# wustl-cig/FLAIR

Measured on AMD Instinct MI355X. Metric: restored frames/sec at 256x256, 16-frame clip, 250-step DDIM, higher is better.
Workload: dtype bf16

## Files before the change

flair_amd/csrc/conv.hip:

```cpp
#include <type_traits>

#include "common.h"
#include "mfma_tile.h"

namespace {

struct ConvArgs {
    const void* x[4];
    int segC[4];
    int segLd[4];
    int nseg;
    const void* w;
    const float* bias;
    const void* res0;
    const void* res1;
    int res0Ld, res1Ld;
    void* y;
    int yLd;
    int T, H, W;
    int KT, KH, KW;
    int Cout, CinTot;
    int act;
    float outScale;
    long P;
    int nPixTiles, nCoTiles;
    int tFast;
    unsigned segBytes[4];
    unsigned wBytes;
    float* part;
    int splitK;
    const float* fbias;
    int fbiasLd;
    int stride;
    int tapShift;
    int reflect;
    float actParam;
    int actPeriod;
    int Hin, Win;
    int esz;
};

__device__ __forceinline__ int lds_off(int row, int chunk) {
    return row * 64 + ((chunk ^ ((row >> 2) & 3)) << 4);
}

__device__ __forceinline__ int staged_row(int id) {
    const int g = id >> 3;
    return (g >> 2) * 8 + (g & 3) + 4 * ((id >> 2) & 1);
}

template <typename E>
__device__ __forceinline__ void store_quad(const ConvArgs& a, long p, int co, float v0, float v1, float v2, float v3) {
    if (co >= a.Cout) return;
    float v[4] = {v0, v1, v2, v3};
    if (a.bias) {
        const float4 b = *reinterpret_cast<const float4*>(a.bias + co);
// ... 187 lines not shown
        const unsigned cofs = (unsigned)(cb * BKE) * ESZ;
#pragma unroll
        for (int i = 0; i < HI; ++i) {
            const unsigned off = hpix[i] >= 0 ? (unsigned)hpix[i] * ld + cofs + hq[i] : FLAIR_OOB;
            hr[i] = buf_load16(xr, off);
        }
        const unsigned kofs = (unsigned)((dt + pt) * 9 * a.CinTot + segOff + cb * BKE) * ESZ;
#pragma unroll
        for (int i = 0; i < WI; ++i) wr[i] = buf_load16(wrs, woff[i] == FLAIR_OOB ? FLAIR_OOB : woff[i] + kofs);
    };
    auto advance = [&]() {
        ++cb;
        if (cb * BKE >= a.segC[seg]) {
            cb = 0;
            segOff += a.segC[seg];
            if (++seg >= a.nseg) {
                seg = 0;
                segOff = 0;
                ++dt;
                while (dt <= pt && !dt_valid(dt)) ++dt;
            }
        }
    };
    auto write_lds = [&](const uint4 (&hr)[HI], const uint4 (&wr)[WI]) {
#pragma unroll
        for (int i = 0; i < HI; ++i) {
            const int id = i * NT + tid;
            const int row = staged_row(id);
            if (row < HALO_ROWS) *reinterpret_cast<uint4*>(sh + row * PITCH + (id & 3) * 16) = hr[i];
        }
#pragma unroll
        for (int i = 0; i < WI; ++i) {
            const int id = i * NT + tid;
            if (id < W_PIECES) *reinterpret_cast<uint4*>(sw + staged_row(id) * PITCH + (id & 3) * 16) = wr[i];
        }
    };
    int nValidDt = 0;
    for (int d = -pt; d <= pt; ++d) nValidDt += dt_valid(d) ? 1 : 0;
    const int nch = nValidDt * (a.CinTot / BKE);

    f32x16 acc[RPW][2];
#pragma unroll
    for (int j = 0; j < RPW; ++j)
#pragma unroll
        for (int i = 0; i < 2; ++i)
#pragma unroll
            for (int r = 0; r < 16; ++r) acc[j][i][r] = 0.f;

    auto compute = [&]() {
        const char* hb = sh + ((wave * RPW * HW_) + lr) * PITCH;
        const char* wb0 = sw + (lr * 9) * PITCH;
        const char* wb1 = sw + ((lr + 32) * 9) * PITCH;
        uint4 fa0[2][2], fa1[2][2], fb[2][RPW][2];
        auto load_tap = [&](int set, int tap9) {
// ... 221 lines not shown
    auto issue = [&]() {
        const unsigned ld = (unsigned)a.segLd[seg] * ESZ;
        const char* frame = reinterpret_cast<const char*>(a.x[seg]) + (size_t)(t + dt) * a.H * a.W * ld;
        const __amdgpu_buffer_rsrc_t xr = make_rsrc(frame, a.segBytes[seg]);
        const unsigned cofs = (unsigned)(cb * BKE) * ESZ;
#pragma unroll
        for (int i = 0; i < HI; ++i)
            hreg[i] = buf_load16(xr, hpix[i] >= 0 ? (unsigned)hpix[i] * ld + cofs + hq[i] : FLAIR_OOB);
        const unsigned kofs = (unsigned)((dt + pt) * 9 * a.CinTot + segOff + cb * BKE) * ESZ;
#pragma unroll
        for (int i = 0; i < WI; ++i) wreg[i] = buf_load16(wrs, woff[i] == FLAIR_OOB ? FLAIR_OOB : woff[i] + kofs);
        ++cb;
        if (cb * BKE >= a.segC[seg]) {
            cb = 0;
            segOff += a.segC[seg];
            if (++seg >= a.nseg) {
                seg = 0;
                segOff = 0;
                ++dt;
                while (dt <= pt && !dt_valid(dt)) ++dt;
            }
        }
    };
    auto write_lds = [&](int stage) {
        char* sh = smem + stage * STAGE_BYTES;
        char* sw = sh + HALO_BYTES;
#pragma unroll
        for (int i = 0; i < HI; ++i) {
            const int id = i * NT + tid;
            const int row = staged_row(id);
            if (row < HALO_ROWS) *reinterpret_cast<uint4*>(sh + row * PITCH + (id & 3) * 16) = hreg[i];
        }
#pragma unroll
        for (int i = 0; i < WI; ++i) {
            const int id = i * NT + tid;
            if (id < W_PIECES) *reinterpret_cast<uint4*>(sw + staged_row(id) * PITCH + (id & 3) * 16) = wreg[i];
        }
    };
    int nValidDt = 0;
    for (int d = -pt; d <= pt; ++d) nValidDt += dt_valid(d) ? 1 : 0;
    const int nch = nValidDt * (a.CinTot / BKE);

    f32x16 acc[2];
#pragma unroll
    for (int i = 0; i < 2; ++i)
#pragma unroll
        for (int r = 0; r < 16; ++r) acc[i][r] = 0.f;

    const int ck = 16 * Mma<E>::chunk(kh2, lh);
    auto compute = [&](int stage) {
        const char* sh = smem + stage * STAGE_BYTES;
        const char* hb = sh + ((rp * HW_) + lr) * PITCH + ck;
        const char* wb0 = sh + HALO_BYTES + (lr * 9) * PITCH + ck;
        uint4 fa[2][2], fb[2];
        auto load_tap = [&](int set, int tap9) {
            const int kh = tap9 / 3, kw = tap9 % 3;
// ... 134 lines not shown
    constexpr int KSTEPS = 2;
    constexpr int TH = NW * RPW, HWP = 34;
    constexpr int HALO_ROWS = (TH + 2) * HWP;
    constexpr int HALO_INSTR = (HALO_ROWS + 15) / 16;
    constexpr int W_INSTR = 64 * 9 / 16;
    constexpr int HALO_BYTES = HALO_INSTR * 1024;
    constexpr int STAGE_BYTES = HALO_BYTES + W_INSTR * 1024;
    constexpr int NSLOT = (HALO_INSTR + W_INSTR + NW - 1) / NW;
    constexpr int BIAS_OFF = NSTAGE * STAGE_BYTES + NW * 1024;
    extern __shared__ __attribute__((aligned(16))) char smem[];

    const int tid = threadIdx.x, lane = tid & 63;
    const int wave = __builtin_amdgcn_readfirstlane(tid >> 6);
    const int lr = lane & 31, lh = lane >> 5;
    const int taps = a.KT * 9, pt = a.KT / 2;
    const int chunksPerTap = a.CinTot / 32;
    const int H = a.H, W = a.W, T = a.T;

    const int xcd = blockIdx.x & 7, slot = blockIdx.x >> 3, slotsPerXcd = gridDim.x >> 3;
    const int tilesW = W / 32, tilesH = H / TH, nCoTiles = a.nCoTiles;
    auto tile_at = [&](int i, DmaTile& tl) -> bool {
        const int inXcd = slot + i * slotsPerXcd;
        const int id = xcd * tilesPerXcd + inXcd;
        if (inXcd >= tilesPerXcd || id >= nTiles) return false;
        int rest = id;
        tl.co0 = (rest % nCoTiles) * 64;
        rest /= nCoTiles;
        if (a.tFast) {
            tl.t = rest % T;
            rest /= T;
            tl.w0 = (rest % tilesW) * 32;
// ... 35 lines not shown
    const u32x4_t wdesc = make_desc(a.w, a.wBytes);
    struct Walk {
        int dt, seg, cb, segOff, j;
    };
    auto dt_at = [&](int t, int j) { return a.tFast ? (j + a.KT * T - t) % a.KT - pt : j - pt; };
    auto walk_first = [&](int t, Walk& wk) {
        wk.j = 0; wk.seg = 0; wk.cb = 0; wk.segOff = 0;
        while (wk.j < a.KT && (unsigned)(t + dt_at(t, wk.j)) >= (unsigned)T) ++wk.j;
        wk.dt = dt_at(t, wk.j);
    };
    auto walk_next = [&](int t, Walk& wk) {
        ++wk.cb;
        if (wk.cb * 32 >= a.segC[wk.seg]) {
            wk.cb = 0;
            wk.segOff += a.segC[wk.seg];
            if (++wk.seg >= a.nseg) {
                wk.seg = 0;
                wk.segOff = 0;
                ++wk.j;
                while (wk.j < a.KT && (unsigned)(t + dt_at(t, wk.j)) >= (unsigned)T) ++wk.j;
                wk.dt = dt_at(t, wk.j);
            }
        }
    };
    auto chunks_of = [&](int t) {
        int n = 0;
        for (int d = -pt; d <= pt; ++d) n += (unsigned)(t + d) < (unsigned)T ? 1 : 0;
        return n * chunksPerTap;
    };
    auto issue = [&](const DmaTile& tl, const Walk& wk, int stage) {
        const unsigned ld = (unsigned)a.segLd[wk.seg] * 2u;
// ... 338 lines not shown
    using E = bf16_t;
    constexpr int NW = 8, HWP = 34;
    constexpr int HINSTR = 22, HIMG = HINSTR * 1024, WINSTR = 36, SLOT = WINSTR * 1024;
    constexpr int HR = 3, WR = 2;
    constexpr int RING = HR * HIMG, BIAS = RING + WR * SLOT;
    constexpr int NH = (HINSTR + NW - 1) / NW, NWS = (WINSTR + NW - 1) / NW;
    extern __shared__ __attribute__((aligned(16))) char smem[];
    const int tid = threadIdx.x, lane = tid & 63;
    const int wave = __builtin_amdgcn_readfirstlane(tid >> 6);
    const int lr = lane & 31, lh = lane >> 5;
    const int lrow = lane >> 2, lchunk = lane & 3;
    const int tilesW = a.W / 32, perFrame = tilesW * (a.H / 8);
    const int bid = xcd_remap(blockIdx.x, gridDim.x);
    const int t = bid / perFrame, tile = bid - t * perFrame;
    const int h0 = (tile / tilesW) * 8, w0 = (tile % tilesW) * 32;
    const int nS = a.CinTot / 32;

    const u32x4_t wdesc = make_desc(a.w, a.wBytes);
    const u32x4_t bdesc = make_desc(a.bias, a.bias ? (unsigned)a.Cout * 4u : 0u);
    dma16(bdesc, (unsigned)(lane * 16), (unsigned)BIAS);
    unsigned hpix[NH], hpiece[NH];
#pragma unroll
    for (int i = 0; i < NH; ++i) dma_halo_coords((wave * NH + i) % HINSTR, lrow, lchunk, 10, h0, w0, a.H, a.W, hpix[i], hpiece[i]);
    unsigned wlane[NWS];
#pragma unroll
    for (int i = 0; i < NWS; ++i) {
        const int id = (wave * NWS + i) % WINSTR;
        const int row = id * 16 + lrow, tap9 = row >> 6, co = row & 63;
        wlane[i] = co < a.Cout ? (unsigned)((co * 9 + tap9) * a.CinTot) * 2u + (unsigned)((lchunk ^ ((co >> 2) & 3)) << 4) : FLAIR_OOB;
    }
    int hseg = 0, hcb = 0;
    auto issue_halo = [&](int slot) {
        const unsigned ld = (unsigned)a.segLd[hseg] * 2u;
        const u32x4_t xdesc = make_desc(reinterpret_cast<const char*>(a.x[hseg]) + (size_t)t * a.H * a.W * ld, a.segBytes[hseg]);
        const unsigned cofs = (unsigned)(hcb * 64);
#pragma unroll
        for (int i = 0; i < NH; ++i) {
            const int k = (wave * NH + i) % HINSTR;
            dma16(xdesc, hpix[i] == 0xffffffffu ? FLAIR_OOB : hpix[i] * ld + cofs + hpiece[i], (unsigned)(slot * HIMG + k * 1024));
        }
        if (++hcb * 32 >= a.segC[hseg]) {
            hcb = 0;
            ++hseg;
        }
    };
    auto issue_w = [&](int s_) {
#pragma unroll
        for (int i = 0; i < NWS; ++i) {
            const int id = (wave * NWS + i) % WINSTR;
            dma16(wdesc, wlane[i] == FLAIR_OOB ? FLAIR_OOB : wlane[i] + (unsigned)(s_ * 64), (unsigned)(RING + (s_ % WR) * SLOT + id * 1024));
        }
    };
    issue_halo(0);
    issue_w(0);
    if (nS > 1) {
        issue_halo(1);
        issue_w(1);
    }
    if (nS > 2) issue_halo(2);

    unsigned aoff[2], boff[3][2];
    dma_frag_offsets(lr, lh, wave * HWP, aoff, boff);
    f32x16 acc[2];
    auto compute = [&](int wslot, int hslot) { dma_tap_loop(smem + RING + wslot * SLOT, smem + hslot * HIMG, aoff, boff, acc, dma_no_hook{}); };

    const long prow = ((long)t * a.H + h0 + wave) * a.W + w0;
// ... 111 lines not shown
        xvalid[i] = p < a.P;
        if (!xvalid[i]) p = 0;
        int w_ = (int)(p % a.W);
        long q = p / a.W;
        xw[i] = w_;
        xh[i] = (int)(q % a.H);
        xt[i] = (int)(q / a.H);
    }
    const int taps = a.KT * a.KH * a.KW;
    const int pt = a.KT / 2, ph = a.KH / 2, pw = a.KW / 2;
    const int tFirst = (int)(p0 / ((long)a.H * a.W));
    const int tileFrames = (int)((TP + (long)a.H * a.W - 1) / ((long)a.H * a.W)) + 1;

    uint4 xreg[PD][XR], wreg[PD][WR];

    const int nkAll = taps * (a.CinTot / BKE);
    const int ks0 = (int)((long)blockIdx.y * nkAll / a.splitK);
    const int ks1 = (int)((long)(blockIdx.y + 1) * nkAll / a.splitK);
    int tap = ks0 / (a.CinTot / BKE), seg = 0, cb = ks0 % (a.CinTot / BKE), segOff = 0;
    while (cb * BKE >= a.segC[seg]) {
        cb -= a.segC[seg] / BKE;
        segOff += a.segC[seg];
        ++seg;
    }
    int dw = tap % a.KW - pw, dh = (tap / a.KW) % a.KH - ph, dt = tap / (a.KW * a.KH) - pt;

    const __amdgpu_buffer_rsrc_t wrs = make_rsrc(a.w, a.wBytes);
    constexpr unsigned ESZ = sizeof(E);
    auto issue_loads = [&](int set) {
        const int ld = a.segLd[seg];
        int fb = tFirst + dt;
        fb = fb < 0 ? 0 : (fb >= a.T ? a.T - 1 : fb);
        int nfr = a.T - fb;
        if (nfr > tileFrames) nfr = tileFrames;
        const size_t frameBytes = (size_t)a.Hin * a.Win * ld * ESZ;
        const __amdgpu_buffer_rsrc_t xr =
            make_rsrc(reinterpret_cast<const char*>(a.x[seg]) + fb * frameBytes, (unsigned)(nfr * frameBytes));
        const int coff = cb * BKE + chunk * VEC;
// ... 11 lines not shown
            xreg[set][i] = buf_load16(xr, off);
        }
        const unsigned kofs = (unsigned)(tap * a.CinTot + segOff + coff) * ESZ;
#pragma unroll
        for (int j = 0; j < WR; ++j) {
            const int n = co0 + srow + RPP * j;
            wreg[set][j] = buf_load16(wrs, n < a.Cout ? (unsigned)(n * taps * a.CinTot) * ESZ + kofs : FLAIR_OOB);
        }
    };
    auto advance = [&]() {
        ++cb;
        if (cb * BKE >= a.segC[seg]) {
            cb = 0;
            segOff += a.segC[seg];
            ++seg;
            if (seg >= a.nseg) {
                seg = 0;
                segOff = 0;
                ++tap;
                ++dw;
                if (dw > pw) {
                    dw = -pw;
                    ++dh;
                    if (dh > ph) {
                        dh = -ph;
                        ++dt;
                    }
                }
            }
        }
// ... 4 lines not shown
        for (int j = 0; j < WR; ++j)
            *reinterpret_cast<uint4*>(base + loff(srow + RPP * j, chunk)) = wreg[set][j];
#pragma unroll
        for (int i = 0; i < XR; ++i)
            *reinterpret_cast<uint4*>(base + TC * ROWB + loff(srow + RPP * i, chunk)) = xreg[set][i];
    };

    f32x16 acc[FC][FP];
#pragma unroll
    for (int i = 0; i < FC; ++i)
#pragma unroll
        for (int j = 0; j < FP; ++j)
#pragma unroll
            for (int r = 0; r < 16; ++r) acc[i][j][r] = 0.f;

    const int nk = ks1 - ks0;
    const int lr = lane & 31, lh = lane >> 5;

#pragma unroll
    for (int u = 0; u < PD; ++u)
        if (u < nk) {
            issue_loads(u);
            advance();
        }
    write_lds(0, 0);
    __syncthreads();

    for (int ks = 0; ks < nk; ks += PD) {
#pragma unroll
        for (int u = 0; u < PD; ++u) {
            const int k = ks + u;
            if (k >= nk) break;
            const int cur = k & 1;
            if (k + PD < nk) {
                issue_loads(u);
                advance();
            }
            const char* wb = smem + cur * BUF;
            const char* xb = wb + TC * ROWB;
#pragma unroll
// ... 215 lines not shown

extern "C" int flair_conv_nhwc(const flair_conv_params* p, const void* const* x, const void* w,
                               const float* bias, const float* frame_bias, const void* res0, const void* res1,
                               void* y, void* workspace, size_t workspace_bytes, hipStream_t stream) {
    FLAIR_CHECK(p && x && w && y, "flair_conv_nhwc: null argument");
    FLAIR_CHECK_DTYPE("flair_conv_nhwc", p->dtype);
    FLAIR_CHECK(p->nseg >= 1 && p->nseg <= 4, "flair_conv_nhwc: nseg %d not in 1..4", p->nseg);
    FLAIR_CHECK(p->T > 0 && p->H > 0 && p->W > 0 && p->Cout > 0, "flair_conv_nhwc: empty shape");
    FLAIR_CHECK((p->KT & 1) && (p->KH & 1) && (p->KW & 1), "flair_conv_nhwc: kernel taps must be odd");
    FLAIR_CHECK(p->Cout % 4 == 0, "flair_conv_nhwc: Cout %d must be a multiple of 4", p->Cout);
    const int bke = p->dtype == FLAIR_BF16 ? 32 : 16;
    const int esz = p->dtype == FLAIR_BF16 ? 2 : 4;
    ConvArgs a{};
    fill_geometry(a, p);
    for (int i = 0; i < p->nseg; ++i) {
        FLAIR_CHECK(x[i], "flair_conv_nhwc: segment %d is null", i);
        FLAIR_CHECK(p->seg_c[i] > 0 && p->seg_c[i] % bke == 0,
                    "flair_conv_nhwc: segment %d has %d channels; must be a multiple of %d", i, p->seg_c[i], bke);
        FLAIR_CHECK(p->seg_ld[i] >= p->seg_c[i] && (p->seg_ld[i] * esz) % 16 == 0 &&
                        ((uintptr_t)x[i]) % 16 == 0,
                    "flair_conv_nhwc: segment %d stride/alignment", i);
        a.x[i] = x[i];
        a.segC[i] = p->seg_c[i];
        a.segLd[i] = p->seg_ld[i];
        const unsigned long long bytes = (unsigned long long)p->H * p->W * p->seg_ld[i] * esz;
        FLAIR_CHECK(bytes < 0x40000000ull, "flair_conv_nhwc: one frame of segment %d spans %llu bytes (limit 1 GiB)",
                    i, bytes);
        a.segBytes[i] = (unsigned)bytes;
    }
    {
        const unsigned long long wb = (unsigned long long)p->Cout * p->KT * p->KH * p->KW * a.CinTot * esz;
        FLAIR_CHECK(wb < 0x80000000ull, "flair_conv_nhwc: weights span %llu bytes (limit 2 GiB)", wb);
    }
    const int gran = (p->dtype == FLAIR_BF16 && p->Cout % 8 != 0) ? 8 : 16;
    FLAIR_CHECK(p->y_ld >= p->Cout && (p->y_ld * esz) % gran == 0 && ((uintptr_t)y) % 16 == 0,
                "flair_conv_nhwc: output stride/alignment (y_ld = %d: >= Cout = %d, a multiple of %d bytes; y 16-byte aligned)",
                p->y_ld, p->Cout, gran);
    FLAIR_CHECK(!res0 || (p->res_ld[0] >= p->Cout && (p->res_ld[0] * esz) % gran == 0 && ((uintptr_t)res0) % gran == 0),
// ... 55 lines not shown
```

flair_amd/csrc/dcn.hip:

```cpp


#include "common.h"
#include "mfma_tile.h"

namespace {

struct DcnArgs {
    const void* x[2];
    int xLd[2];
    int Cin;
    const void* raw; int rawLd;
    const float* flow1;
    const float* flow2;
    const void* w;
    const float* bias;
    void* y; int yLd;
    int F, H, W, Cout, G;
    float maxMag;
    int activated;
    long P;
    unsigned xBytes[2], rawBytes, wBytes;
};

template <int CPR>
// ... 86 lines not shown
            const int px = id / slabPieces, pc = id - px * slabPieces;
            if (px < TP) *reinterpret_cast<uint4*>(sraw + ((tap & 1) * TP + px) * rawPitch + pc * 16) = reg[j];
        }
    };
    auto stage_raw = [&](int tap) {
        uint4 reg[RAWR];
        raw_issue(tap, reg);
        raw_write(tap, reg);
    };

    const int cpg = a.Cin / G;
    int cpgShift = 0;
    while ((1 << cpgShift) < cpg) ++cpgShift;
    const int halfC = a.Cin / 2;
    const int cbPerTap = a.Cin / BKE;
    const int nk = 9 * cbPerTap;
    const size_t fo0 = ONEFRAME ? (size_t)pf * a.H * a.W * a.xLd[0] * ESZ : 0, fo1 = ONEFRAME ? (size_t)pf * a.H * a.W * a.xLd[1] * ESZ : 0;
    const __amdgpu_buffer_rsrc_t xr0 = make_rsrc(reinterpret_cast<const char*>(a.x[0]) + fo0, a.xBytes[0]);
    const __amdgpu_buffer_rsrc_t xr1 = make_rsrc(reinterpret_cast<const char*>(a.x[1]) + fo1, a.xBytes[1]);
    const __amdgpu_buffer_rsrc_t wrs = make_rsrc(a.w, a.wBytes);
    const unsigned frameBase = (unsigned)pf * a.H * a.W;

    struct Regs {
        uint4 c[4];
        uint4 w[WR];
        float wt[4];
    } rs[PFD];

    unsigned wrow[WR];
#pragma unroll
    for (int j = 0; j < WR; ++j) {
        const int id = tid + j * NT;
        const int n = id / CPR, ch = id % CPR;
        wrow[j] = n < a.Cout && n < TC ? (unsigned)(n * 9 * a.Cin + ch * VEC) * ESZ : FLAIR_OOB;
// ... 50 lines not shown
            r.wt[1] = (1.f - ay) * ax * mk;
            r.wt[2] = ay * (1.f - ax) * mk;
            r.wt[3] = ay * ax * mk;
            const unsigned o00 = (unsigned)mul_i24(
                                     (int)frameBase + mul_i24(y0, a.W) + x0, (int)ld) + coff;
            const bool yok0 = pvalid && (unsigned)y0 < (unsigned)a.H, yok1 = pvalid && (unsigned)(y0 + 1) < (unsigned)a.H;
            const bool xok0 = (unsigned)x0 < (unsigned)a.W, xok1 = (unsigned)(x0 + 1) < (unsigned)a.W;
            r.c[0] = buf_load16(xr, yok0 && xok0 ? o00 : FLAIR_OOB);
            r.c[1] = buf_load16(xr, yok0 && xok1 ? o00 + ld : FLAIR_OOB);
            r.c[2] = buf_load16(xr, yok1 && xok0 ? o00 + rowStep : FLAIR_OOB);
            r.c[3] = buf_load16(xr, yok1 && xok1 ? o00 + rowStep + ld : FLAIR_OOB);
        }
        const unsigned wk = (unsigned)(tap * a.Cin + cb * BKE) * ESZ;
#pragma unroll
        for (int j = 0; j < WR; ++j) r.w[j] = buf_load16(wrs, wrow[j] == FLAIR_OOB ? FLAIR_OOB : wrow[j] + wk);
        if (++icb == cbPerTap) {
            icb = 0;
            ++itap;
            if (++ikw == 3) {
                ikw = 0;
                ++ikh;
            }
        }
    };
    auto blend_and_stage = [&](const Regs& r, int buf) {
        char* base = stile + buf * BUF;
        uint4 outv;
        if constexpr (sizeof(E) == 2 && DOT2) {
            typedef __attribute__((ext_vector_type(2))) __bf16 bf16x2_t;
            const bf16x2_t w01 = __builtin_bit_cast(bf16x2_t, cvt_pk_bf16(r.wt[0], r.wt[1]));
            const bf16x2_t w23 = __builtin_bit_cast(bf16x2_t, cvt_pk_bf16(r.wt[2], r.wt[3]));
// ... 54 lines not shown
            const int id = tid + j * NT;
            if (id < TC * CPR) *reinterpret_cast<uint4*>(base + tile_off<CPR>(id / CPR, id % CPR)) = r.w[j];
        }
    };

    f32x16 acc[PAIRS];
#pragma unroll
    for (int i = 0; i < PAIRS; ++i)
#pragma unroll
        for (int r = 0; r < 16; ++r) acc[i][r] = 0.f;

    constexpr int LEAD = PFD + 1;
    int stageTap = 0;
    {
        uint4 r0[RAWR], r1[RAWR];
        const bool two = cbPerTap - LEAD < 0;
        raw_issue(0, r0);
        if (two) raw_issue(1, r1);
        raw_write(0, r0);
        if (two) raw_write(1, r1);
        stageTap = two ? 2 : 1;
    }
    int stageAt = stageTap * cbPerTap - LEAD;
    __syncthreads();
    auto mfma_step = [&](int buf) {
        const char* wb = stile + buf * BUF;
        const char* xb = wb + TC * CPR * 16;
#pragma unroll
        for (int i = 0; i < PAIRS; ++i) {
            const int pair = KSPLIT > 1 ? wave % NPAIR : wave * PAIRS + i;
            const int kpart = KSPLIT > 1 ? wave / NPAIR : 0;
            const int pfrag = pair % NPF, cf = pair / NPF;
#pragma unroll
            for (int kk = 0; kk < KSUB; ++kk) {
                const int ks = kpart * KSUB + kk;
                uint4 af[2], bf[2];
#pragma unroll
                for (int h = 0; h < 2; ++h) {
                    const int ch = ks * 4 + Mma<E>::chunk(h, lh);
                    bf[h] = *reinterpret_cast<const uint4*>(xb + tile_off<CPR>(pfrag * 32 + lr, ch));
                    af[h] = *reinterpret_cast<const uint4*>(wb + tile_off<CPR>(cf * 32 + lr, ch));
                }
                Mma<E>::run(af, bf, acc[i]);
            }
        }
    };
#pragma unroll
    for (int u = 0; u < PFD - 1; ++u)
        if (u < nk) issue(rs[u]);
    constexpr int UNR = 2 * PFD;
    for (int k = 0; k < nk; k += UNR) {
#pragma unroll
        for (int u = 0; u < UNR; ++u) {
            if (k + u < nk) {
                if (k + u + PFD - 1 < nk) issue(rs[(u + PFD - 1) % PFD]);
                blend_and_stage(rs[u % PFD], u & 1);
                __syncthreads();
                mfma_step(u & 1);
                if (k + u == stageAt && stageTap < 9) {
                    stage_raw(stageTap);
                    ++stageTap;
                    stageAt += cbPerTap;
                }
            }
        }
    }
    if constexpr (KSPLIT > 1) {
        __syncthreads();
        float* red = reinterpret_cast<float*>(stile);
        const int pair0 = wave % NPAIR, kpart0 = wave / NPAIR;
        if (kpart0 > 0) {
            float* dst = red + ((kpart0 - 1) * NPAIR + pair0) * 64 * 16 + lane * 16;
#pragma unroll
            for (int r = 0; r < 16; r += 4)
                *reinterpret_cast<float4*>(dst + r) = make_float4(acc[0][r], acc[0][r + 1], acc[0][r + 2], acc[0][r + 3]);
        }
        __syncthreads();
// ... 62 lines not shown
                pk.y = pack2bf(v[2], v[3]);
                *reinterpret_cast<uint2*>(dst) = pk;
            }
        }
    }
}

}

template <typename E, int NCF, int NPF, int TPP, int OFFS, bool ONEFRAME>
static int launch_dcn_v(const DcnArgs& a0, hipStream_t stream) {
    DcnArgs a = a0;
    if (ONEFRAME) {
        const unsigned long long half = a.Cin / 2, hw = (unsigned long long)a.H * a.W;
        a.xBytes[0] = (unsigned)(((hw - 1) * a.xLd[0] + half) * sizeof(E));
        a.xBytes[1] = (unsigned)(((hw - 1) * a.xLd[1] + half) * sizeof(E));
    }
    constexpr int NT = 32 * NPF * TPP, TP = 32 * NPF, TC = 32 * NCF;
    const int rawPitch = (OFFS == 2 ? (3 * a.G * (int)sizeof(E) + 15) & ~15 : 3 * a.G * (int)sizeof(E)) + 16;
    const size_t lds = (size_t)2 * TP * rawPitch + 2 * (TC + TP) * TPP * 16;
    static LdsAttrOnce attr;
    {
        const hipError_t e = flair_max_lds_once(attr, reinterpret_cast<const void*>(&dcn_kernel<E, NCF, NPF, TPP, OFFS, ONEFRAME>));
        FLAIR_CHECK(e == hipSuccess, "flair_dcn_align: hipFuncSetAttribute: %s", hipGetErrorString(e));
    }
    hipLaunchKernelGGL((dcn_kernel<E, NCF, NPF, TPP, OFFS, ONEFRAME>), dim3(cdiv(a.P, TP)), dim3(NT), lds, stream, a);
    FLAIR_LAUNCH_CHECK();
    return FLAIR_OK;
}

template <typename E, int NCF, int NPF, int TPP>
// ... 39 lines not shown
        DcnArgs a = a0;
        a.Cout = p->Cout - co0 < t.tc ? p->Cout - co0 : t.tc;
        a.w = static_cast<const char*>(a0.w) + (size_t)co0 * 9 * p->Cin * esz;
        a.bias = a0.bias ? a0.bias + co0 : nullptr;
        a.y = static_cast<char*>(a0.y) + (size_t)co0 * esz;
        a.wBytes = (unsigned)((unsigned long long)a.Cout * 9 * p->Cin * esz);
        const int rc = p->dtype == FLAIR_BF16 ? launch_dcn_vqfr<bf16_t>(p, a, stream) : launch_dcn_vqfr<float>(p, a, stream);
        if (rc != FLAIR_OK) return rc;
    }
    return FLAIR_OK;
}

extern "C" int flair_dcn_align(const flair_dcn_params* p, const void* x0, const void* x1, const void* raw,
                               const float* flow1, const float* flow2, const void* w, const float* bias, void* y,
                               hipStream_t stream) {
    FLAIR_CHECK(p && x0 && x1 && raw && w && y, "flair_dcn_align: null argument");
    FLAIR_CHECK_DTYPE("flair_dcn_align", p->dtype);
    FLAIR_CHECK(p->raw_activated >= 0 && p->raw_activated <= 2, "flair_dcn_align: raw_activated = %d (0, 1 or 2)", p->raw_activated);
    const bool vqfr = p->raw_activated == 2;
    FLAIR_CHECK(!vqfr || (!flow1 && !flow2), "flair_dcn_align: raw_activated = 2 takes no flows");
    const int vec = p->dtype == FLAIR_BF16 ? 8 : 4;
    const int bke = vqfr ? vqfr_tile(p).bke : vec * (p->Cout <= 64 && p->dtype != FLAIR_BF16 ? 4 : 8);
    const int esz = p->dtype == FLAIR_BF16 ? 2 : 4;
    const int cpg = p->G > 0 ? p->Cin / p->G : 0;
    FLAIR_CHECK(p->G > 0 && (p->G % 8 == 0 || (vqfr && p->G == 4)) && p->G <= 16 && p->Cin % p->G == 0 && cpg % vec == 0 &&
                    (cpg & (cpg - 1)) == 0 && (p->Cin / 2) % bke == 0 && (!vqfr || p->Cin <= 1024),
                "flair_dcn_align: Cin=%d G=%d not supported", p->Cin, p->G);
    FLAIR_CHECK(p->Cout > 0 && p->Cout % 4 == 0 && (vqfr ? p->Cout <= 1024 : p->Cout <= 128) && p->raw_ld >= 27 * p->G &&
                    (p->raw_ld * esz) % 16 == 0,
                "flair_dcn_align: Cout = %d (a multiple of 4, <= 128; <= 1024 with raw_activated = 2) / raw_ld = %d (>= 27 G, "
                "16-byte granular)", p->Cout, p->raw_ld);
    FLAIR_CHECK(p->x_ld[0] >= p->Cin / 2 && p->x_ld[1] >= p->Cin / 2 && (p->x_ld[0] * esz) % 16 == 0 &&
                    (p->x_ld[1] * esz) % 16 == 0 && ((uintptr_t)x0) % 16 == 0 && ((uintptr_t)x1) % 16 == 0 &&
                    ((uintptr_t)raw) % 16 == 0 && p->y_ld >= p->Cout,
                "flair_dcn_align: strides/alignment (x_ld = %d, %d: >= Cin / 2 = %d, 16-byte granular; x0, x1, raw 16-byte "
                "aligned; y_ld = %d >= Cout = %d)", p->x_ld[0], p->x_ld[1], p->Cin / 2, p->y_ld, p->Cout);
    DcnArgs a;
    a.x[0] = x0; a.x[1] = x1; a.xLd[0] = p->x_ld[0]; a.xLd[1] = p->x_ld[1];
    a.Cin = p->Cin; a.raw = raw; a.rawLd = p->raw_ld; a.flow1 = flow1; a.flow2 = flow2;
    a.w = w; a.bias = bias; a.y = y; a.yLd = p->y_ld;
    a.F = p->F; a.H = p->H; a.W = p->W; a.Cout = p->Cout; a.G = p->G; a.maxMag = p->max_residue_magnitude;
    a.activated = p->raw_activated;
    a.P = (long)p->F * p->H * p->W;
    const unsigned long long half = p->Cin / 2;
    const unsigned long long b0 = ((unsigned long long)(a.P - 1) * p->x_ld[0] + half) * esz;
    const unsigned long long b1 = ((unsigned long long)(a.P - 1) * p->x_ld[1] + half) * esz;
    const unsigned long long br = ((unsigned long long)(a.P - 1) * p->raw_ld + 27 * p->G) * esz;
    const unsigned long long by = (unsigned long long)a.P * p->y_ld * esz;
    FLAIR_CHECK(b0 < 0x80000000ull && b1 < 0x80000000ull && br < 0x80000000ull && by < 0x80000000ull, "flair_dcn_align: tensor spans >= 2 GiB");
    FLAIR_CHECK(a.P + 2l * p->W + 2 < (1l << 23) && (long)p->x_ld[0] * esz < (1l << 23) && (long)p->x_ld[1] * esz < (1l << 23),
                "flair_dcn_align: F*H*W = %ld pixels (limit 2^23 per call: call per frame)", a.P);
    a.xBytes[0] = (unsigned)b0; a.xBytes[1] = (unsigned)b1; a.rawBytes = (unsigned)((br + 15) / 16 * 16);
    a.wBytes = (unsigned)((unsigned long long)p->Cout * 9 * p->Cin * esz);
    if (vqfr) return dcn_vqfr(p, a, stream);
    if (p->dtype == FLAIR_BF16) {
        if (p->Cout > 64) {
            if (a.P >= 64 * 256 && (p->Cin / 2) % 128 == 0) return launch_dcn<bf16_t, 4, 2, 16>(a, stream);
            if (a.P >= 64 * 256) return launch_dcn<bf16_t, 4, 2, 8>(a, stream);
            return launch_dcn<bf16_t, 4, 1, 8>(a, stream);
        }
        return a.P >= 128 * 512 ? launch_dcn<bf16_t, 2, 4, 8>(a, stream) : launch_dcn<bf16_t, 2, 2, 8>(a, stream);
    }
    return p->Cout <= 64 ? launch_dcn<float, 2, 2, 4>(a, stream) : launch_dcn<float, 4, 1, 8>(a, stream);
}
```

flair_amd/guided_diffusion/unet_new.py:

```python
import math

import torch
import torch.nn as nn

from .. import ops
from .clip_model import ClipModel
from .nn_new import conv_nd, linear, normalization, zero_module
from .packing import LinearStack, dev_f32, pack_w, packed_conv, pk_int, run_conv

A = ops


class PlaceHolder(nn.Module):

    def __init__(self, module):
        super().__init__()
        self.wrapped_module = module


LazyReshaper2D = LazyReshaper3D = PlaceHolder


class TemporalWrapper(PlaceHolder):
    """unet_new.py:50-59 (skipped when ``enable_cross_frames`` is False)."""
# ... 319 lines not shown
        ka = ops.k_align(ctx.dtype)
        k3 = (1, 3, 3)
        G = self.deform_align[name].deform_groups
        mag = float(self.deform_align[name].max_residue_magnitude)
        store = ctx.flows.get("_prop") if isinstance(ctx.flows, dict) else None
        key = (name, H, W, ctx.dtype, ka)
        cached = store.get(key) if store is not None else None
        fill = [] if (cached is None and store is not None) else None
        prop, prev2 = zero_c, None
        for i, idx in enumerate(order):
            cur = hidden[idx:idx + 1]
            if i > 0:
                flow_n1 = flows[flow_idx[i]:flow_idx[i] + 1]
                cond_n1 = torch.empty_like(zero_c)
                second = i > 1
                feat_n2 = prev2 if second else zero_c
                cond_n2 = torch.empty_like(zero_c) if second else zero_c
                if cached is not None:
                    flow_n2, flowpad = cached[i - 1]
                    ops.vsrpp_warp2(prop, feat_n2 if second else None, flow_n1, flow_n2, cond_n1, cond_n2 if second else None)
                else:
                    flowpad = torch.zeros((1, H, W, ka), dtype=ctx.dtype, device=ctx.device)
                    flow_n2 = torch.empty_like(flow_n1) if second else None
                    ops.vsrpp_prep(prop, feat_n2 if second else None, flow_n1,
                                   flows[flow_idx[i - 1]:flow_idx[i - 1] + 1] if second else None,
                                   cond_n1, cond_n2 if second else None, flow_n2, flowpad)
                    if fill is not None:
                        fill.append((flow_n2, flowpad))
                o = ops.conv([cond_n1, cur, cond_n2, flowpad], pk_a["w0"], pk_a["b0"], c, k3, act=A.ACT_LRELU01)
                if c == 64 and ops.chain_supported(o, c):
                    o = ops.conv_chain(o, pk_a["w2"], pk_a["b2"], A.ACT_LRELU01, pk_a["w4"], pk_a["b4"],
                                       A.ACT_LRELU01, c, c)
                else:
                    o = ops.conv(o, pk_a["w2"], pk_a["b2"], c, k3, act=A.ACT_LRELU01)
                    o = ops.conv(o, pk_a["w4"], pk_a["b4"], c, k3, act=A.ACT_LRELU01)
                if c == 64 and ops.chain_supported(o, c) and W % 32 == 0:
                    raw = ops.conv_chain(o, None, None, A.ACT_NONE, pk_a["w6"], pk_a["b6"], A.ACT_DCN_OFFSETS, c, 27 * G,
                                         act_param=mag, act_period=3 * G)
                else:
                    raw = ops.conv(o, pk_a["w6"], pk_a["b6"], 27 * G, k3, act=A.ACT_DCN_OFFSETS, act_param=mag,
                                   act_period=3 * G)
                aligned = ops.dcn_align(prop, feat_n2, raw, flow_n1, flow_n2, pk_a["wd"], pk_a["bd"], c,
                                        groups=G, max_mag=mag, raw_activated=True)

            else:
                aligned = zero_c
            segs = [cur] + [o_[idx:idx + 1] for o_ in others] + [aligned]
            new = run_trunk(pk_t, segs, c, extra_res=aligned, out=dest[idx:idx + 1], out_scale=weight)
            if wmaps is not None:
                ops.scale_pixels(new, wmaps[idx])
            prev2, prop = (prop if i > 0 else None), new
        if fill is not None:
            store[key] = fill
        return dest

    def run(self, ctx, hidden):
        T, H, W, c = hidden.shape
        flows_forward, flows_backward = ctx.flows[W]
        weight, wmaps = 1.0, None
        vw = ctx.vsrpp_weights
        if isinstance(vw, (float, int)):
# ... 289 lines not shown
```

flair_amd/ops.py:

```python
import ctypes

import torch

from ._header import STRUCTS
from ._lib import ACT_DCN_OFFSETS, ACT_GELU, ACT_LRELU01, ACT_LRELU02, ACT_NONE, ACT_RELU, ACT_SILU, ConvParams, call, dtype_code, lib
from ._lib import check, ptr, stream

__all__ = ["conv", "conv_chain", "group_norm", "nchw_to_clip", "clip_to_nchw", "timestep_embedding", "linear",
           "qkv_attention", "temporal_attention", "flow_warp", "flow_compose", "resize",
           "dcn_align", "dcn_raw_permutation", "scale_pixels", "predict_xstart", "sampler_update",
           "ACT_NONE", "ACT_RELU", "ACT_LRELU01", "ACT_SILU", "ACT_DCN_OFFSETS", "ACT_LRELU02", "ACT_GELU"]


GnParams, SamplerCoefs, AttnParams = STRUCTS["flair_gn_params"], STRUCTS["flair_sampler_coefs"], STRUCTS["flair_attn_params"]
TAttnParams, DcnParams, ChainParams = STRUCTS["flair_tattn_params"], STRUCTS["flair_dcn_params"], STRUCTS["flair_chain_params"]


def _ld(t):
    assert t.dim() == 4 and t.stride(3) == 1, "clip tensors are (T,H,W,C) with C innermost"
    ld = t.stride(2)
    assert t.stride(1) == ld * t.shape[2] and (t.shape[0] == 1 or t.stride(0) == ld * t.shape[1] * t.shape[2]), \
        "clip tensor must be dense over (T,H,W)"
    return ld

# ... 13 lines not shown


def conv(xs, weight, bias, cout, kernel, *, out=None, act=ACT_NONE, res0=None, res1=None,
         out_scale=1.0, stride=1, frame_bias=None, act_param=0.0, act_period=0, asym_pad=False, reflect_pad=False):
    if isinstance(xs, torch.Tensor):
        xs = [xs]
    x0 = xs[0]
    T, H, W, _ = x0.shape
    p = ConvParams()
    p.dtype = dtype_code(x0)
    p.T, p.H, p.W = T, H, W
    p.KT, p.KH, p.KW = kernel
    p.Cout = cout
    p.nseg = len(xs)
    arr = (ctypes.c_void_p * 4)()
    for i, x in enumerate(xs):
        assert x.dtype == x0.dtype and x.shape[:3] == x0.shape[:3]
        p.seg_c[i] = x.shape[3]
        p.seg_ld[i] = _ld(x)
        arr[i] = x.data_ptr()
    p.stride = stride
    p.asym_pad = asym_pad
    p.reflect_pad = reflect_pad
    p.frame_bias_ld = frame_bias.stride(0) if frame_bias is not None else 0
    if frame_bias is not None:
        assert frame_bias.dtype == torch.float32 and frame_bias.stride(1) == 1 and frame_bias.shape[0] == T
    Ho, Wo = (H + stride - 1) // stride, (W + stride - 1) // stride
    if out is None:
        out = torch.empty((T, Ho, Wo, cout), dtype=x0.dtype, device=x0.device)
    assert tuple(out.shape[:3]) == (T, Ho, Wo) and out.shape[3] >= cout and out.dtype == x0.dtype
    p.y_ld = _ld(out)
    p.res_ld[0] = _ld(res0) if res0 is not None else 0
    p.res_ld[1] = _ld(res1) if res1 is not None else 0
    p.act = act
    p.act_param, p.act_period = act_param, act_period
    p.out_scale = out_scale
    assert weight.dtype == x0.dtype and weight.is_contiguous()
    e0 = _prof_begin()
    wsb = _conv_ws_bytes(p)
    ws = _workspace(wsb, x0.device, "conv") if wsb else None

    def launch(_keep=xs):
        call.flair_conv_nhwc(ctypes.byref(p), arr, weight, _dense(bias), frame_bias, res0, res1, out, ws, wsb)
    launch()
    if e0 is not None:
        cin = sum(x.shape[3] for x in xs)
        taps = kernel[0] * kernel[1] * kernel[2]
        esz = x0.element_size()
        flops = 2.0 * T * Ho * Wo * cout * cin * taps
        nbytes = esz * (cin * T * H * W + cout * T * Ho * Wo * (1 + (res0 is not None) + (res1 is not None))
                        + cout * taps * cin)
        _prof_end(e0, ("conv", lib().flair_conv_variant(ctypes.byref(p))), x0.dtype, flops, nbytes, launch,
                  ("conv", T, H, W, tuple(x.shape[3] for x in xs), cout, tuple(kernel), stride, act,
                   res0 is not None, res1 is not None, frame_bias is not None))
    return out


PROFILE = None


def _prof_begin():
    if PROFILE is None:
        return None
    e0 = torch.cuda.Event(enable_timing=True)
    e0.record()
    return e0


def _prof_end(e0, family, dtype, flops, nbytes, replay=None, sig=None):
    e1 = torch.cuda.Event(enable_timing=True)
# ... 263 lines not shown
    perm = torch.empty(27 * G, dtype=torch.long)
    for k in range(9):
        for g in range(G):
            for e in range(2):
                perm[3 * G * k + 2 * g + e] = 2 * (g * 9 + k) + e
            perm[3 * G * k + 2 * G + g] = 18 * G + g * 9 + k
    return perm


def dcn_align(x0, x1, raw, flow1, flow2, weight, bias, cout, *, groups=16, max_mag=10.0, out=None, raw_activated=False):
    F_, H, W, ch = x0.shape
    p = DcnParams()
    p.dtype = dtype_code(x0)
    p.F, p.H, p.W = F_, H, W
    p.Cin, p.Cout, p.G = 2 * ch, cout, groups
    p.x_ld[0], p.x_ld[1] = _ld(x0), _ld(x1)
    p.raw_ld = _ld(raw)
    if out is None:
        out = torch.empty((F_, H, W, cout), dtype=x0.dtype, device=x0.device)
    p.y_ld = _ld(out)
    p.max_residue_magnitude = max_mag
    p.raw_activated = raw_activated
    e0 = _prof_begin()

    def launch():
        call.flair_dcn_align(ctypes.byref(p), x0, x1, raw, flow1, flow2, weight, _dense(bias), out)
    launch()
    if e0 is not None:
        px = F_ * H * W
        _prof_end(e0, ("dcn", cout), x0.dtype, px * (2.0 * 9 * 2 * ch * cout + 9.0 * 2 * ch * 8),
                  x0.element_size() * px * (2 * ch + 27 * groups + cout), launch,
                  ("dcn", F_, H, W, ch, cout, groups, flow2 is not None))
    return out


def dcn_pack(x, raw, weight, bias, cout, *, groups, out=None):
    c = x.shape[3]
    assert c % 2 == 0
    return dcn_align(x[..., :c // 2], x[..., c // 2:], raw, None, None, weight, bias, cout, groups=groups, out=out,
                     raw_activated=2)


def scale_pixels(x, wmap):
    T, H, W, C = x.shape
    call.flair_scale_pixels(x, dtype_code(x), _ld(x), C, T * H * W, _dense(wmap))
    return x

# ... 740 lines not shown
```

Before: 0.8474.

## Skip zero-valued input segments in conv and DCN kernels instead of multiplying zeros

Conv kernels now accept null input segments and skip their K-chunks. Channel counts are derived from the weight shape, and the split-K ranges are recomputed over the present chunks only. The DCN align kernel runs half the K loop when the second input is absent. The VSR propagation passes None instead of zero tensors for the first-step neighbours and the aligned feature. This avoids loading and running MFMA on all-zero channels. The cost is more complex K-iteration and split-K bookkeeping, plus a prologue change to raw staging in DCN.

New measurement: 0.8522, median of 6. Within noise of the previous version (+0.6%).

```diff
diff --git a/flair_amd/csrc/conv.hip b/flair_amd/csrc/conv.hip
--- a/flair_amd/csrc/conv.hip
+++ b/flair_amd/csrc/conv.hip
@@ -20,6 +20,7 @@
     int T, H, W;
     int KT, KH, KW;
     int Cout, CinTot;
+    int CinAct;
     int act;
     float outScale;
     long P;
@@ -40,6 +41,13 @@
     int esz;
 };
 
+__device__ __forceinline__ void skip_absent(const ConvArgs& a, int& seg, int& segOff) {
+    while (seg < a.nseg && !a.x[seg]) {
+        segOff += a.segC[seg];
+        ++seg;
+    }
+}
+
 __device__ __forceinline__ int lds_off(int row, int chunk) {
     return row * 64 + ((chunk ^ ((row >> 2) & 3)) << 4);
 }
@@ -257,7 +265,9 @@
         if (cb * BKE >= a.segC[seg]) {
             cb = 0;
             segOff += a.segC[seg];
-            if (++seg >= a.nseg) {
+            ++seg;
+            skip_absent(a, seg, segOff);
+            if (seg >= a.nseg) {
                 seg = 0;
                 segOff = 0;
                 ++dt;
@@ -280,7 +290,7 @@
     };
     int nValidDt = 0;
     for (int d = -pt; d <= pt; ++d) nValidDt += dt_valid(d) ? 1 : 0;
-    const int nch = nValidDt * (a.CinTot / BKE);
+    const int nch = nValidDt * (a.CinAct / BKE);
 
     f32x16 acc[RPW][2];
 #pragma unroll
@@ -532,7 +542,9 @@
         if (cb * BKE >= a.segC[seg]) {
             cb = 0;
             segOff += a.segC[seg];
-            if (++seg >= a.nseg) {
+            ++seg;
+            skip_absent(a, seg, segOff);
+            if (seg >= a.nseg) {
                 seg = 0;
                 segOff = 0;
                 ++dt;
@@ -557,7 +569,7 @@
     };
     int nValidDt = 0;
     for (int d = -pt; d <= pt; ++d) nValidDt += dt_valid(d) ? 1 : 0;
-    const int nch = nValidDt * (a.CinTot / BKE);
+    const int nch = nValidDt * (a.CinAct / BKE);
 
     f32x16 acc[2];
 #pragma unroll
@@ -722,7 +734,7 @@
     const int wave = __builtin_amdgcn_readfirstlane(tid >> 6);
     const int lr = lane & 31, lh = lane >> 5;
     const int taps = a.KT * 9, pt = a.KT / 2;
-    const int chunksPerTap = a.CinTot / 32;
+    const int chunksPerTap = a.CinAct / 32;
     const int H = a.H, W = a.W, T = a.T;
 
     const int xcd = blockIdx.x & 7, slot = blockIdx.x >> 3, slotsPerXcd = gridDim.x >> 3;
@@ -788,7 +800,9 @@
         if (wk.cb * 32 >= a.segC[wk.seg]) {
             wk.cb = 0;
             wk.segOff += a.segC[wk.seg];
-            if (++wk.seg >= a.nseg) {
+            ++wk.seg;
+            skip_absent(a, wk.seg, wk.segOff);
+            if (wk.seg >= a.nseg) {
                 wk.seg = 0;
                 wk.segOff = 0;
                 ++wk.j;
@@ -1157,7 +1171,7 @@
     const int bid = xcd_remap(blockIdx.x, gridDim.x);
     const int t = bid / perFrame, tile = bid - t * perFrame;
     const int h0 = (tile / tilesW) * 8, w0 = (tile % tilesW) * 32;
-    const int nS = a.CinTot / 32;
+    const int nS = a.CinAct / 32;
 
     const u32x4_t wdesc = make_desc(a.w, a.wBytes);
     const u32x4_t bdesc = make_desc(a.bias, a.bias ? (unsigned)a.Cout * 4u : 0u);
@@ -1172,7 +1186,18 @@
         const int row = id * 16 + lrow, tap9 = row >> 6, co = row & 63;
         wlane[i] = co < a.Cout ? (unsigned)((co * 9 + tap9) * a.CinTot) * 2u + (unsigned)((lchunk ^ ((co >> 2) & 3)) << 4) : FLAIR_OOB;
     }
-    int hseg = 0, hcb = 0;
+    auto k_next = [&](int& seg, int& cb, int& full) {
+        ++full;
+        if (++cb * 32 >= a.segC[seg]) {
+            cb = 0;
+            ++seg;
+            while (seg < a.nseg && !a.x[seg]) {
+                full += a.segC[seg] / 32;
+                ++seg;
+            }
+        }
+    };
+    int hseg = 0, hcb = 0, hfull = 0, wseg = 0, wcb = 0, wfull = 0;
     auto issue_halo = [&](int slot) {
         const unsigned ld = (unsigned)a.segLd[hseg] * 2u;
         const u32x4_t xdesc = make_desc(reinterpret_cast<const char*>(a.x[hseg]) + (size_t)t * a.H * a.W * ld, a.segBytes[hseg]);
@@ -1182,17 +1207,15 @@
             const int k = (wave * NH + i) % HINSTR;
             dma16(xdesc, hpix[i] == 0xffffffffu ? FLAIR_OOB : hpix[i] * ld + cofs + hpiece[i], (unsigned)(slot * HIMG + k * 1024));
         }
-        if (++hcb * 32 >= a.segC[hseg]) {
-            hcb = 0;
-            ++hseg;
-        }
+        k_next(hseg, hcb, hfull);
     };
     auto issue_w = [&](int s_) {
 #pragma unroll
         for (int i = 0; i < NWS; ++i) {
             const int id = (wave * NWS + i) % WINSTR;
-            dma16(wdesc, wlane[i] == FLAIR_OOB ? FLAIR_OOB : wlane[i] + (unsigned)(s_ * 64), (unsigned)(RING + (s_ % WR) * SLOT + id * 1024));
-        }
+            dma16(wdesc, wlane[i] == FLAIR_OOB ? FLAIR_OOB : wlane[i] + (unsigned)(wfull * 64), (unsigned)(RING + (s_ % WR) * SLOT + id * 1024));
+        }
+        k_next(wseg, wcb, wfull);
     };
     issue_halo(0);
     issue_w(0);
@@ -1334,14 +1357,31 @@
 
     uint4 xreg[PD][XR], wreg[PD][WR];
 
-    const int nkAll = taps * (a.CinTot / BKE);
+    const int cpt = a.CinTot / BKE;
+    const int nkAll = taps * cpt;
     const int ks0 = (int)((long)blockIdx.y * nkAll / a.splitK);
     const int ks1 = (int)((long)(blockIdx.y + 1) * nkAll / a.splitK);
-    int tap = ks0 / (a.CinTot / BKE), seg = 0, cb = ks0 % (a.CinTot / BKE), segOff = 0;
-    while (cb * BKE >= a.segC[seg]) {
-        cb -= a.segC[seg] / BKE;
+    auto present_before = [&](int ks) {
+        const int c = ks % cpt;
+        int n = ks / cpt * (a.CinAct / BKE), beg = 0;
+        for (int i = 0; i < a.nseg; ++i) {
+            const int len = a.segC[i] / BKE;
+            if (a.x[i] && c > beg) n += c - beg < len ? c - beg : len;
+            beg += len;
+        }
+        return n;
+    };
+    int tap = ks0 / cpt, seg = 0, cb = ks0 % cpt, segOff = 0;
+    while (seg < a.nseg && (!a.x[seg] || cb * BKE >= a.segC[seg])) {
+        cb = cb * BKE >= a.segC[seg] ? cb - a.segC[seg] / BKE : 0;
         segOff += a.segC[seg];
         ++seg;
+    }
+    if (seg >= a.nseg) {
+        seg = 0;
+        cb = 0;
+        segOff = 0;
+        ++tap;
     }
     int dw = tap % a.KW - pw, dh = (tap / a.KW) % a.KH - ph, dt = tap / (a.KW * a.KH) - pt;
 
@@ -1383,6 +1423,7 @@
             cb = 0;
             segOff += a.segC[seg];
             ++seg;
+            skip_absent(a, seg, segOff);
             if (seg >= a.nseg) {
                 seg = 0;
                 segOff = 0;
@@ -1417,7 +1458,7 @@
 #pragma unroll
             for (int r = 0; r < 16; ++r) acc[i][j][r] = 0.f;
 
-    const int nk = ks1 - ks0;
+    const int nk = present_before(ks1) - present_before(ks0);
     const int lr = lane & 31, lh = lane >> 5;
 
 #pragma unroll
@@ -1426,7 +1467,7 @@
             issue_loads(u);
             advance();
         }
-    write_lds(0, 0);
+    if (nk > 0) write_lds(0, 0);
     __syncthreads();
 
     for (int ks = 0; ks < nk; ks += PD) {
@@ -1672,14 +1713,16 @@
     ConvArgs a{};
     fill_geometry(a, p);
     for (int i = 0; i < p->nseg; ++i) {
-        FLAIR_CHECK(x[i], "flair_conv_nhwc: segment %d is null", i);
+        FLAIR_CHECK(x[i] || i > 0, "flair_conv_nhwc: segment %d is null", i);
         FLAIR_CHECK(p->seg_c[i] > 0 && p->seg_c[i] % bke == 0,
                     "flair_conv_nhwc: segment %d has %d channels; must be a multiple of %d", i, p->seg_c[i], bke);
+        a.segC[i] = p->seg_c[i];
+        if (!x[i]) continue;
+        a.CinAct += p->seg_c[i];
         FLAIR_CHECK(p->seg_ld[i] >= p->seg_c[i] && (p->seg_ld[i] * esz) % 16 == 0 &&
                         ((uintptr_t)x[i]) % 16 == 0,
                     "flair_conv_nhwc: segment %d stride/alignment", i);
         a.x[i] = x[i];
-        a.segC[i] = p->seg_c[i];
         a.segLd[i] = p->seg_ld[i];
         const unsigned long long bytes = (unsigned long long)p->H * p->W * p->seg_ld[i] * esz;
         FLAIR_CHECK(bytes < 0x40000000ull, "flair_conv_nhwc: one frame of segment %d spans %llu bytes (limit 1 GiB)",
diff --git a/flair_amd/csrc/dcn.hip b/flair_amd/csrc/dcn.hip
--- a/flair_amd/csrc/dcn.hip
+++ b/flair_amd/csrc/dcn.hip
@@ -124,10 +124,11 @@
     while ((1 << cpgShift) < cpg) ++cpgShift;
     const int halfC = a.Cin / 2;
     const int cbPerTap = a.Cin / BKE;
-    const int nk = 9 * cbPerTap;
+    const int cbRun = a.x[1] ? cbPerTap : cbPerTap / 2;
+    const int nk = 9 * cbRun;
     const size_t fo0 = ONEFRAME ? (size_t)pf * a.H * a.W * a.xLd[0] * ESZ : 0, fo1 = ONEFRAME ? (size_t)pf * a.H * a.W * a.xLd[1] * ESZ : 0;
     const __amdgpu_buffer_rsrc_t xr0 = make_rsrc(reinterpret_cast<const char*>(a.x[0]) + fo0, a.xBytes[0]);
-    const __amdgpu_buffer_rsrc_t xr1 = make_rsrc(reinterpret_cast<const char*>(a.x[1]) + fo1, a.xBytes[1]);
+    const __amdgpu_buffer_rsrc_t xr1 = make_rsrc(a.x[1] ? reinterpret_cast<const char*>(a.x[1]) + fo1 : nullptr, a.xBytes[1]);
     const __amdgpu_buffer_rsrc_t wrs = make_rsrc(a.w, a.wBytes);
     const unsigned frameBase = (unsigned)pf * a.H * a.W;
 
@@ -208,7 +209,7 @@
         const unsigned wk = (unsigned)(tap * a.Cin + cb * BKE) * ESZ;
 #pragma unroll
         for (int j = 0; j < WR; ++j) r.w[j] = buf_load16(wrs, wrow[j] == FLAIR_OOB ? FLAIR_OOB : wrow[j] + wk);
-        if (++icb == cbPerTap) {
+        if (++icb == cbRun) {
             icb = 0;
             ++itap;
             if (++ikw == 3) {
@@ -293,14 +294,14 @@
     int stageTap = 0;
     {
         uint4 r0[RAWR], r1[RAWR];
-        const bool two = cbPerTap - LEAD < 0;
+        const bool two = cbRun - LEAD < 0;
         raw_issue(0, r0);
         if (two) raw_issue(1, r1);
         raw_write(0, r0);
         if (two) raw_write(1, r1);
         stageTap = two ? 2 : 1;
     }
-    int stageAt = stageTap * cbPerTap - LEAD;
+    int stageAt = stageTap * cbRun - LEAD;
     __syncthreads();
     auto mfma_step = [&](int buf) {
         const char* wb = stile + buf * BUF;
@@ -325,8 +326,15 @@
         }
     };
 #pragma unroll
-    for (int u = 0; u < PFD - 1; ++u)
+    for (int u = 0; u < PFD - 1; ++u) {
         if (u < nk) issue(rs[u]);
+        if (u - (PFD - 1) == stageAt && stageTap < 9) {
+            __syncthreads();
+            stage_raw(stageTap);
+            ++stageTap;
+            stageAt += cbRun;
+        }
+    }
     constexpr int UNR = 2 * PFD;
     for (int k = 0; k < nk; k += UNR) {
 #pragma unroll
@@ -339,7 +347,7 @@
                 if (k + u == stageAt && stageTap < 9) {
                     stage_raw(stageTap);
                     ++stageTap;
-                    stageAt += cbPerTap;
+                    stageAt += cbRun;
                 }
             }
         }
@@ -432,7 +440,7 @@
     if (ONEFRAME) {
         const unsigned long long half = a.Cin / 2, hw = (unsigned long long)a.H * a.W;
         a.xBytes[0] = (unsigned)(((hw - 1) * a.xLd[0] + half) * sizeof(E));
-        a.xBytes[1] = (unsigned)(((hw - 1) * a.xLd[1] + half) * sizeof(E));
+        a.xBytes[1] = a.x[1] ? (unsigned)(((hw - 1) * a.xLd[1] + half) * sizeof(E)) : 0u;
     }
     constexpr int NT = 32 * NPF * TPP, TP = 32 * NPF, TC = 32 * NCF;
     const int rawPitch = (OFFS == 2 ? (3 * a.G * (int)sizeof(E) + 15) & ~15 : 3 * a.G * (int)sizeof(E)) + 16;
@@ -502,7 +510,7 @@
 extern "C" int flair_dcn_align(const flair_dcn_params* p, const void* x0, const void* x1, const void* raw,
                                const float* flow1, const float* flow2, const void* w, const float* bias, void* y,
                                hipStream_t stream) {
-    FLAIR_CHECK(p && x0 && x1 && raw && w && y, "flair_dcn_align: null argument");
+    FLAIR_CHECK(p && x0 && raw && w && y, "flair_dcn_align: null argument");
     FLAIR_CHECK_DTYPE("flair_dcn_align", p->dtype);
     FLAIR_CHECK(p->raw_activated >= 0 && p->raw_activated <= 2, "flair_dcn_align: raw_activated = %d (0, 1 or 2)", p->raw_activated);
     const bool vqfr = p->raw_activated == 2;
@@ -518,13 +526,13 @@
                     (p->raw_ld * esz) % 16 == 0,
                 "flair_dcn_align: Cout = %d (a multiple of 4, <= 128; <= 1024 with raw_activated = 2) / raw_ld = %d (>= 27 G, "
                 "16-byte granular)", p->Cout, p->raw_ld);
-    FLAIR_CHECK(p->x_ld[0] >= p->Cin / 2 && p->x_ld[1] >= p->Cin / 2 && (p->x_ld[0] * esz) % 16 == 0 &&
-                    (p->x_ld[1] * esz) % 16 == 0 && ((uintptr_t)x0) % 16 == 0 && ((uintptr_t)x1) % 16 == 0 &&
+    FLAIR_CHECK(p->x_ld[0] >= p->Cin / 2 && (!x1 || p->x_ld[1] >= p->Cin / 2) && (p->x_ld[0] * esz) % 16 == 0 &&
+                    (!x1 || (p->x_ld[1] * esz) % 16 == 0) && ((uintptr_t)x0) % 16 == 0 && ((uintptr_t)x1) % 16 == 0 &&
                     ((uintptr_t)raw) % 16 == 0 && p->y_ld >= p->Cout,
                 "flair_dcn_align: strides/alignment (x_ld = %d, %d: >= Cin / 2 = %d, 16-byte granular; x0, x1, raw 16-byte "
                 "aligned; y_ld = %d >= Cout = %d)", p->x_ld[0], p->x_ld[1], p->Cin / 2, p->y_ld, p->Cout);
     DcnArgs a;
-    a.x[0] = x0; a.x[1] = x1; a.xLd[0] = p->x_ld[0]; a.xLd[1] = p->x_ld[1];
+    a.x[0] = x0; a.x[1] = x1; a.xLd[0] = p->x_ld[0]; a.xLd[1] = x1 ? p->x_ld[1] : 0;
     a.Cin = p->Cin; a.raw = raw; a.rawLd = p->raw_ld; a.flow1 = flow1; a.flow2 = flow2;
     a.w = w; a.bias = bias; a.y = y; a.yLd = p->y_ld;
     a.F = p->F; a.H = p->H; a.W = p->W; a.Cout = p->Cout; a.G = p->G; a.maxMag = p->max_residue_magnitude;
@@ -532,11 +540,11 @@
     a.P = (long)p->F * p->H * p->W;
     const unsigned long long half = p->Cin / 2;
     const unsigned long long b0 = ((unsigned long long)(a.P - 1) * p->x_ld[0] + half) * esz;
-    const unsigned long long b1 = ((unsigned long long)(a.P - 1) * p->x_ld[1] + half) * esz;
+    const unsigned long long b1 = x1 ? ((unsigned long long)(a.P - 1) * p->x_ld[1] + half) * esz : 0;
     const unsigned long long br = ((unsigned long long)(a.P - 1) * p->raw_ld + 27 * p->G) * esz;
     const unsigned long long by = (unsigned long long)a.P * p->y_ld * esz;
     FLAIR_CHECK(b0 < 0x80000000ull && b1 < 0x80000000ull && br < 0x80000000ull && by < 0x80000000ull, "flair_dcn_align: tensor spans >= 2 GiB");
-    FLAIR_CHECK(a.P + 2l * p->W + 2 < (1l << 23) && (long)p->x_ld[0] * esz < (1l << 23) && (long)p->x_ld[1] * esz < (1l << 23),
+    FLAIR_CHECK(a.P + 2l * p->W + 2 < (1l << 23) && (long)p->x_ld[0] * esz < (1l << 23) && (long)a.xLd[1] * esz < (1l << 23),
                 "flair_dcn_align: F*H*W = %ld pixels (limit 2^23 per call: call per frame)", a.P);
     a.xBytes[0] = (unsigned)b0; a.xBytes[1] = (unsigned)b1; a.rawBytes = (unsigned)((br + 15) / 16 * 16);
     a.wBytes = (unsigned)((unsigned long long)p->Cout * 9 * p->Cin * esz);
diff --git a/flair_amd/guided_diffusion/unet_new.py b/flair_amd/guided_diffusion/unet_new.py
--- a/flair_amd/guided_diffusion/unet_new.py
+++ b/flair_amd/guided_diffusion/unet_new.py
@@ -357,17 +357,17 @@
                 flow_n1 = flows[flow_idx[i]:flow_idx[i] + 1]
                 cond_n1 = torch.empty_like(zero_c)
                 second = i > 1
-                feat_n2 = prev2 if second else zero_c
-                cond_n2 = torch.empty_like(zero_c) if second else zero_c
+                feat_n2 = prev2 if second else None
+                cond_n2 = torch.empty_like(zero_c) if second else None
                 if cached is not None:
                     flow_n2, flowpad = cached[i - 1]
-                    ops.vsrpp_warp2(prop, feat_n2 if second else None, flow_n1, flow_n2, cond_n1, cond_n2 if second else None)
+                    ops.vsrpp_warp2(prop, feat_n2, flow_n1, flow_n2, cond_n1, cond_n2)
                 else:
                     flowpad = torch.zeros((1, H, W, ka), dtype=ctx.dtype, device=ctx.device)
                     flow_n2 = torch.empty_like(flow_n1) if second else None
-                    ops.vsrpp_prep(prop, feat_n2 if second else None, flow_n1,
+                    ops.vsrpp_prep(prop, feat_n2, flow_n1,
                                    flows[flow_idx[i - 1]:flow_idx[i - 1] + 1] if second else None,
-                                   cond_n1, cond_n2 if second else None, flow_n2, flowpad)
+                                   cond_n1, cond_n2, flow_n2, flowpad)
                     if fill is not None:
                         fill.append((flow_n2, flowpad))
                 o = ops.conv([cond_n1, cur, cond_n2, flowpad], pk_a["w0"], pk_a["b0"], c, k3, act=A.ACT_LRELU01)
@@ -387,7 +387,7 @@
                                         groups=G, max_mag=mag, raw_activated=True)
 
             else:
-                aligned = zero_c
+                aligned = None
             segs = [cur] + [o_[idx:idx + 1] for o_ in others] + [aligned]
             new = run_trunk(pk_t, segs, c, extra_res=aligned, out=dest[idx:idx + 1], out_scale=weight)
             if wmaps is not None:
diff --git a/flair_amd/ops.py b/flair_amd/ops.py
--- a/flair_amd/ops.py
+++ b/flair_amd/ops.py
@@ -51,9 +51,12 @@
     p.Cout = cout
     p.nseg = len(xs)
     arr = (ctypes.c_void_p * 4)()
+    widths = _seg_widths(xs, weight)
     for i, x in enumerate(xs):
+        p.seg_c[i] = widths[i]
+        if x is None:
+            continue
         assert x.dtype == x0.dtype and x.shape[:3] == x0.shape[:3]
-        p.seg_c[i] = x.shape[3]
         p.seg_ld[i] = _ld(x)
         arr[i] = x.data_ptr()
     p.stride = stride
@@ -81,16 +84,27 @@
         call.flair_conv_nhwc(ctypes.byref(p), arr, weight, _dense(bias), frame_bias, res0, res1, out, ws, wsb)
     launch()
     if e0 is not None:
-        cin = sum(x.shape[3] for x in xs)
+        cin = sum(x.shape[3] for x in xs if x is not None)
         taps = kernel[0] * kernel[1] * kernel[2]
         esz = x0.element_size()
         flops = 2.0 * T * Ho * Wo * cout * cin * taps
         nbytes = esz * (cin * T * H * W + cout * T * Ho * Wo * (1 + (res0 is not None) + (res1 is not None))
                         + cout * taps * cin)
         _prof_end(e0, ("conv", lib().flair_conv_variant(ctypes.byref(p))), x0.dtype, flops, nbytes, launch,
-                  ("conv", T, H, W, tuple(x.shape[3] for x in xs), cout, tuple(kernel), stride, act,
+                  ("conv", T, H, W, tuple(x.shape[3] if x is not None else 0 for x in xs), cout, tuple(kernel), stride, act,
                    res0 is not None, res1 is not None, frame_bias is not None))
     return out
+
+
+def _seg_widths(xs, weight):
+    widths = [x.shape[3] if x is not None else 0 for x in xs]
+    absent = widths.count(0)
+    if absent:
+        assert xs[0] is not None, "the first input segment must be present"
+        rest = weight.shape[-1] - sum(widths)
+        assert rest > 0 and rest % absent == 0, (weight.shape, widths)
+        widths = [c or rest // absent for c in widths]
+    return widths
 
 
 PROFILE = None
@@ -384,7 +398,7 @@
     p.dtype = dtype_code(x0)
     p.F, p.H, p.W = F_, H, W
     p.Cin, p.Cout, p.G = 2 * ch, cout, groups
-    p.x_ld[0], p.x_ld[1] = _ld(x0), _ld(x1)
+    p.x_ld[0], p.x_ld[1] = _ld(x0), _ld(x1) if x1 is not None else 0
     p.raw_ld = _ld(raw)
     if out is None:
         out = torch.empty((F_, H, W, cout), dtype=x0.dtype, device=x0.device)
@@ -400,7 +414,7 @@
         px = F_ * H * W
         _prof_end(e0, ("dcn", cout), x0.dtype, px * (2.0 * 9 * 2 * ch * cout + 9.0 * 2 * ch * 8),
                   x0.element_size() * px * (2 * ch + 27 * groups + cout), launch,
-                  ("dcn", F_, H, W, ch, cout, groups, flow2 is not None))
+                  ("dcn", F_, H, W, ch, cout, groups, flow2 is not None, x1 is not None))
     return out
 
 
```
